# JokerYan/MS-GS

Hardware: AMD Instinct MI355X
Metric: Mpixels/s fwd+bwd @1080p, 1M Gaussians; fraction of HBM roofline (higher is better)
Workload: dtype f32

## Files before the change

### include/msgs.h

```cpp
#ifndef MSGS_H_
#define MSGS_H_

#include <stddef.h>
#include <stdint.h>

#ifdef __cplusplus
extern "C" {
#endif

#define MSGS_ABI_VERSION 11

#define MSGS_OK 0
#define MSGS_ERR_INVALID_ARG (-1)
#define MSGS_ERR_CAPACITY (-2)
#define MSGS_ERR_TOO_MANY (-3)
#define MSGS_ERR_SH_DEGREE (-4)
#define MSGS_ERR_INTERNAL (-5)
#define MSGS_ERR_NO_WEIGHT (-6)

#define MSGS_TILE 16

typedef struct msgs_view {
    int32_t image_height;
    int32_t image_width;
// ... 266 lines not shown
                            float* dL_dfeatures_dc, float* dL_dfeatures_rest, void* stream);

int msgs_mark_visible(int32_t P, const float* means3D, const float* viewmatrix,
                      const float* projmatrix, uint8_t* present, void* stream);

int msgs_binning_stats(const msgs_view_t* view, int32_t P, const int32_t* radii,
                       const void* binning, size_t binning_bytes,
                       const void* image_state, size_t image_bytes,
                       void* scratch, size_t scratch_bytes,
                       int64_t* out_host, void* stream);

int msgs_blend_lane_stats(const msgs_view_t* view, const void* geom, size_t geom_bytes, int32_t P, int64_t D,
                          const void* binning, size_t binning_bytes, const void* image_state, size_t image_bytes,
                          void* scratch, size_t scratch_bytes, int64_t* out_host, void* stream);

int msgs_set_deterministic(int32_t on);
int msgs_get_deterministic(void);
size_t msgs_backward_scratch_bytes_deterministic(int32_t P, int64_t D);
size_t msgs_backward_scratch_bytes_deterministic_depth(int32_t P, int64_t D);

int msgs_set_backward_generation(int32_t gen);

int msgs_set_blend_granularity(int32_t mode);

int msgs_set_occlusion(int32_t on);
int msgs_set_depth_sort(int32_t mode);
int msgs_depth_sort_stats(const void* geom, size_t geom_bytes, int32_t P, int64_t* out_host, void* stream);
int msgs_forward_info(int64_t* out_host);
int msgs_occlusion_stats(const void* geom, size_t geom_bytes, int32_t P, int64_t* out_host, void* stream);
int msgs_slab_stats(const void* geom, size_t geom_bytes, int32_t P, int64_t* out_host, void* stream);

int msgs_forward(const msgs_view_t* view, const msgs_gaussians_t* gaussians, int32_t* radii, float* pixel_sizes,
                 void* geom, size_t geom_bytes, void* scratch1, size_t scratch1_bytes, void* binning,
                 size_t binning_bytes, void* scratch2, size_t scratch2_bytes, void* image, size_t image_bytes,
                 float* out_color, float* out_acc_pixel_size, float* out_depth, void* grad_records,
                 size_t grad_records_bytes, int32_t backward_follows, int64_t* num_instances_host, int32_t* stage2_done,
                 const msgs_timing_t* timing, void* stream);

typedef struct msgs_status msgs_status_t;
int msgs_status_create(msgs_status_t** out);
int msgs_status_destroy(msgs_status_t* status);
int msgs_forward_launch(const msgs_view_t* view, const msgs_gaussians_t* gaussians, int32_t* radii, float* pixel_sizes,
                        void* geom, size_t geom_bytes, void* scratch1, size_t scratch1_bytes, void* binning,
                        size_t binning_bytes, void* scratch2, size_t scratch2_bytes, void* image, size_t image_bytes,
                        float* out_color, float* out_acc_pixel_size, float* out_depth, void* grad_records,
                        size_t grad_records_bytes, int32_t backward_follows, msgs_status_t* status,
// ... 226 lines not shown
```

### ms-gs_amd/csrc/api.hip

```cpp
#include "msgs_internal.h"

#include <atomic>
#include <new>

#include <cstring>

using namespace msgs;

namespace {

struct Timer {
    const msgs_timing_t* t;
    hipStream_t s;
    void begin(int k) const { if (t && t->ev[2 * k]) (void)hipEventRecord((hipEvent_t)t->ev[2 * k], s); }
    void end(int k) const { if (t && t->ev[2 * k + 1]) (void)hipEventRecord((hipEvent_t)t->ev[2 * k + 1], s); }
};

inline int check_inputs(const msgs_view_t* v, const msgs_gaussians_t* g) {
    if (!v || !g) return MSGS_ERR_INVALID_ARG;
    if (g->P < 0 || v->image_width <= 0 || v->image_height <= 0) return MSGS_ERR_INVALID_ARG;
    if (!v->bg || !v->viewmatrix || !v->projmatrix || !v->campos) return MSGS_ERR_INVALID_ARG;
    if (g->P > 0 && (!g->means3D || !g->opacities)) return MSGS_ERR_INVALID_ARG;
    if (g->raw_params) {
        if (g->raw_params != 1 && g->raw_params != 2) return MSGS_ERR_INVALID_ARG;
// ... 67 lines not shown
    const Stage2Scratch L(D);
    return L.total + align256(4 * (size_t)(D > 0 ? D : 1));
}
static int64_t tiles_of(int32_t W, int32_t H) { return (int64_t)((W + TILE - 1) / TILE) * ((H + TILE - 1) / TILE); }
size_t msgs_binning_bytes_slab(int64_t D, int32_t W, int32_t H, float fraction) {
    if (!(fraction > 0.f)) return msgs_binning_bytes(D, W, H);
    return msgs_binning_bytes(SlabGeom::ids_needed(D > 0 ? D : 1, (double)fraction, tiles_of(W, H)), W, H);
}
size_t msgs_stage2_scratch_bytes_slab(int64_t D, int32_t W, int32_t H) {
    return msgs_stage2_scratch_bytes((D > 0 ? D : 1) + SLAB_SLACK + 256, W, H);
}
size_t msgs_image_bytes(int32_t W, int32_t H) { return ImageLayout(W, H).total; }
size_t msgs_backward_scratch_bytes(int32_t P) {
    return align256(GRAD_REC_BYTES * (size_t)(P > 0 ? P : 1));
}
size_t msgs_backward_scratch_bytes_deterministic(int32_t P, int64_t D) { return DetScratch(P, D).total; }
size_t msgs_backward_scratch_bytes_deterministic_depth(int32_t P, int64_t D) { return DetScratch(P, D, DET_INST_FLOATS_DEPTH).total; }

static std::atomic<int> g_deterministic{[] { const char* e = getenv("MSGS_DETERMINISTIC"); return (e && e[0] == '1') ? 1 : 0; }()};
int msgs_set_deterministic(int32_t on) { return g_deterministic.exchange(on ? 1 : 0); }
int msgs_get_deterministic(void) { return g_deterministic.load(); }
int msgs_set_backward_generation(int32_t gen) { return set_backward_generation(gen); }
int msgs_set_blend_granularity(int32_t mode) { return set_blend_granularity(mode); }
int msgs_set_occlusion(int32_t on) { return set_occlusion(on); }
int msgs_set_depth_sort(int32_t mode) { return set_depth_sort(mode); }

}

namespace {
struct Stage2Buffers {
    void* binning; size_t binning_bytes;
    void* scratch2; size_t scratch2_bytes;
    void* image; size_t image_bytes;
    float* out_color; float* out_acc_ps; float* out_depth;
    void* grad_records; size_t grad_records_bytes;
    int backward_follows;
};

struct SpecStage2 {
    int64_t capacity;
    Stage2Buffers buf;
    int launched_rc;
};
int forward_stage2_impl(const msgs_view_t* view, const msgs_gaussians_t* g, const void* geom_v, size_t geom_bytes, int64_t D,
                        const Stage2Buffers& b, const msgs_timing_t* timing, void* stream, const uint32_t* D_dev,
                        uint64_t* fb_dev, uint64_t fb_ticket);
// ... 1487 lines not shown
```

### ms-gs_amd/csrc/blend.hip

```cpp
#include "msgs_internal.h"

#include <atomic>
#include <type_traits>

#include <algorithm>

namespace msgs {

namespace {

constexpr int BATCH = 256;
constexpr float ALPHA_MIN = 1.0f / 255.0f;
constexpr float T_MIN = 0.0001f;

struct PairEval { float dxx, dxy, dyy, p; };
__device__ __forceinline__ PairEval eval_pair(float A, float B2, float C, float lo, float dx, float dy) {
#pragma clang fp contract(off)
    PairEval e;
    e.dxx = __fmul_rn(dx, dx);
    e.dxy = __fmul_rn(dx, dy);
    e.dyy = __fmul_rn(dy, dy);
    e.p = __fmaf_rn(A, e.dxx, __fmaf_rn(B2, e.dxy, __fmaf_rn(C, e.dyy, lo)));
    return e;
}
__device__ __forceinline__ float4 doubled_w(const float4& r) { return make_float4(r.x, r.y, r.z, r.w + r.w); }
__device__ __forceinline__ float sign_test_bound(float lo) { return __fmaf_rn(fabsf(lo), 2.4e-7f, lo); }
__device__ __forceinline__ float4 with_bound(const float4& r2, float lo) { return make_float4(r2.x, r2.y, r2.z, sign_test_bound(lo)); }

__device__ __forceinline__ uint32_t quadrant_mask(const float4& r0, float C, float tau2, float tx0, float ty0) {
    if (!(tau2 > -1.0e38f)) return 0xFu;
    uint32_t m = 0;
#pragma unroll
    for (int q = 0; q < 4; ++q) {
        const float x0 = tx0 + (float)((q & 1) * 8), y0 = ty0 + (float)((q >> 1) * 8);
        if (levelset_hits_rect(r0.x, r0.y, r0.z, r0.w, C, tau2, x0, x0 + 7.0f, y0, y0 + 7.0f)) m |= 1u << q;
    }
    return m;
}

__device__ __forceinline__ int swizzled_tile(int bid, int num_tiles) {
    const int per = num_tiles >> 3;
    const int main = per << 3;
    if (bid >= main) return bid;
    return (bid & 7) * per + (bid >> 3);
}

constexpr int CLEAR_INLINE_MIN_TILES = 2048;
__device__ __forceinline__ void clear_slice(uint4* __restrict__ p, size_t n16) {
    if (p == nullptr) return;
// ... 381 lines not shown
                                               grad_acc_t* __restrict__ grad_rec, bool alane, uint32_t aoff) {
    const float outv = cross_row(row_reduce_scatter<DEPTH>(v, v9));
    const uint32_t gid = __builtin_amdgcn_readfirstlane(id());
    grad_acc_t* gdst = grad_rec + (size_t)gid * GRAD_REC_FLOATS;
    if (alane) unsafeAtomicAdd(gdst + aoff, (grad_acc_t)outv);
}
struct BwdPix {
    float T, S, dL0, dL1, dL2, dLd;
    uint32_t last;
};
template <bool ALPHA>
__device__ __forceinline__ void bwd_pix_start_S(BwdPix& st, const ViewParams& vp, bool inside, size_t pix,
                                                const float* dL_dalpha) {
    st.S = vp.bg[0] * st.dL0 + vp.bg[1] * st.dL1 + vp.bg[2] * st.dL2;
    if constexpr (ALPHA) { if (inside) st.S -= dL_dalpha[pix]; }
}
struct PairAlpha { PairEval ev; float a_raw; };
__device__ __forceinline__ PairAlpha pair_alpha(const float4& r0, const float4& r1, float dx, float dy) {
    PairAlpha a;
    a.ev = eval_pair(r0.z, r0.w, r1.x, r1.y, dx, dy);
    a.a_raw = __builtin_amdgcn_exp2f(a.ev.p);
    return a;
}
__device__ __forceinline__ uint64_t pair_valid(const PairAlpha& a, uint32_t pos, uint32_t last, float bound) {
    return __builtin_amdgcn_ballot_w64(pos < last) & __builtin_amdgcn_ballot_w64(a.ev.p <= bound) &
           __builtin_amdgcn_ballot_w64(a.a_raw >= ALPHA_MIN);
}
struct PairGrad { float q, dch; };
template <bool DEPTH, class Z>
__device__ __forceinline__ PairGrad pair_grad(BwdPix& s, const PairAlpha& a, uint64_t validm, const float4& r1, float cb, Z z) {
    const bool valid = __builtin_amdgcn_inverse_ballot_w64(validm);
    const float a_m = valid ? a.a_raw : 0.0f;
    const float alpha_m = fminf(0.99f, a_m);
    const float inv = __builtin_amdgcn_rcpf(1.0f - alpha_m);
    const float Tn = s.T * inv;
    s.T = Tn;
    PairGrad g;
    g.dch = alpha_m * Tn;
    float gi = fmaf(cb, s.dL2, fmaf(r1.w, s.dL1, r1.z * s.dL0));
    if constexpr (DEPTH) gi = fmaf(z(), s.dLd, gi);
    const float sm = gi - s.S;
    const float dL_dalpha = sm * Tn;
    s.S = fmaf(alpha_m, sm, s.S);
    g.q = a_m * dL_dalpha;
    return g;
}
template <bool CROSS_ROW, bool DEPTH = false>
__device__ __forceinline__ void backward_walk(const uint16_t* lp, int cnt, int base, const float4* s_r0, const float4* s_r1,
                                              const float2* s_b, const uint32_t* s_id, float pxf, float pyf, BwdPix& st,
                                              bool alane, uint32_t aoff, grad_acc_t* __restrict__ grad_rec,
                                              const float* s_z = nullptr) {
    for (int j = cnt - 1; j >= 0; --j) {
        const int e = lp[j];
        const float4 r0 = s_r0[e], r1 = s_r1[e];
        const float2 bl = s_b[e];
        const float dx = r0.x - pxf, dy = r0.y - pyf;
// ... 168 lines not shown
        if (b > 0) fetch(base - BATCH);
        __syncthreads();
        int cnt = 0;
#pragma unroll
        for (int c = 0; c < BATCH / 64; ++c) {
            const int e = c * 64 + lane;
            const bool hit = e < n && (uint32_t)(base + e) < wave_last && fine_hit<SB>(s_r0, s_r1, s_tau, e, bx0, by0);
            const uint64_t bal = __ballot(hit);
            if (hit) s_list[w][cnt + __popcll(bal & lt_mask)] = (uint16_t)e;
            cnt += __popcll(bal);
        }
        backward_walk<false, DEPTH>(s_list[w], cnt, base, s_r0, s_r1, s_b, s_id, pxf, pyf, st, alane, aoff, grad_rec, s_z);
    }
}

constexpr int WB = 64;

__device__ __forceinline__ void wave_fence() {
    __builtin_amdgcn_fence(__ATOMIC_RELEASE, "wavefront");
    __builtin_amdgcn_wave_barrier();
    __builtin_amdgcn_fence(__ATOMIC_ACQUIRE, "wavefront");
}

template <bool DEPTH>
__device__ __forceinline__ uint64_t bwd_quad_step(BwdPix& s, BwdSums& v, float* v9, const float4& r0, const float4& r1, float cb,
                                                  float bound, float dx, float dy, uint32_t pos0, float z) {
    const PairAlpha a = pair_alpha(r0, r1, dx, dy);
    const uint64_t validm = pair_valid(a, pos0, s.last, bound);
    const PairGrad g = pair_grad<DEPTH>(s, a, validm, r1, cb, [=] { return z; });
    v.v0 = fmaf(g.q, dx, v.v0); v.v1 = fmaf(g.q, dy, v.v1);
    v.v2 = fmaf(g.q, a.ev.dxx, v.v2); v.v3 = fmaf(g.q, a.ev.dxy, v.v3); v.v4 = fmaf(g.q, a.ev.dyy, v.v4);
    v.v5 += g.q;
    v.v6 = fmaf(g.dch, s.dL0, v.v6); v.v7 = fmaf(g.dch, s.dL1, v.v7); v.v8 = fmaf(g.dch, s.dL2, v.v8);
    if constexpr (DEPTH) *v9 = fmaf(g.dch, s.dLd, *v9);
    return validm;
}

#if defined(MSGS_TRACE_TILES)
__device__ unsigned long long* g_tile_trace = nullptr;
__global__ void trace_set_kernel(unsigned long long* p) { g_tile_trace = p; }
#endif

template <bool COUNT = false, int CH = 3, bool ALPHA = false>
__global__ __launch_bounds__(64) void blend_backward_tile_kernel(ViewParams vp, const GaussRec* __restrict__ rec,
                                                                 const uint32_t* __restrict__ ids,
                                                                 const uint2* __restrict__ ranges,
                                                                 const float* __restrict__ final_T,
                                                                 const uint32_t* __restrict__ n_contrib,
                                                                 const float* __restrict__ dL_dcolor,
                                                                 void* __restrict__ grad_out,
                                                                 const uint32_t* __restrict__ tile_order,
                                                                 const float* __restrict__ dL_ddepth,
                                                                 const float* __restrict__ dL_dalpha) {
    constexpr bool DEPTH = CH == 4;
    __shared__ float4 s_r0[WB], s_r1[WB];
    __shared__ float4 s_bi[WB];
    const int num_tiles = vp.gx * vp.gy;
    const int lane = threadIdx.x;
    int tile = swizzled_tile(blockIdx.x, num_tiles);
    if (tile_order != nullptr) {
        const uint32_t flag = tile_order[num_tiles];
        if (flag == TILE_ORDER_MAGIC) tile = (int)tile_order[tile];
    }
    const int tx = tile % vp.gx, ty = tile / vp.gx;
    const int bx = tx * TILE + (lane & 7), by = ty * TILE + (lane >> 3);
    const float bxf = (float)bx, byf = (float)by;
    const float tx0 = (float)(tx * TILE), ty0 = (float)(ty * TILE);
    const uint2 range = ranges[tile];
    const size_t N = (size_t)vp.W * vp.H;

#if defined(MSGS_TRACE_TILES)
    const unsigned long long trace_t0 = __builtin_amdgcn_s_memrealtime();
#endif
    uint32_t cnt_visits = 0, cnt_steps = 0, cnt_lanes = 0, cnt_hits = 0;
    BwdPix q0, q1, q2, q3;
    uint32_t ql0, ql1, ql2, ql3;
// ... 11 lines not shown
            s.S = vp.bg[0] * s.dL0 + vp.bg[1] * s.dL1 + vp.bg[2] * s.dL2;
            if constexpr (ALPHA) { if (inside) s.S -= dL_dalpha[pix]; }
            s.T = Tf;
            return __builtin_amdgcn_readfirstlane(wave_max_u32(s.last));
        };
        ql0 = init(q0, 0); ql1 = init(q1, 1); ql2 = init(q2, 2); ql3 = init(q3, 3);
    }
    const uint32_t tile_last = max(max(ql0, ql1), max(ql2, ql3));
    const bool alane = IS_ATOMIC_LANE(DEPTH, lane);
    const uint32_t aoff = row_reduce_component<DEPTH>(lane);
    const int xrow16 = (lane ^ 16) << 2, xrow32 = (lane ^ 32) << 2;

    const int nb = ((int)tile_last + WB - 1) / WB;
    float4 n0 = make_float4(0, 0, 0, 0), n1 = n0, n2 = n0;
    uint32_t nid = 0;
    if (nb > 0) {
        const int i0 = (nb - 1) * WB + lane;
        if (i0 < (int)tile_last) { nid = ids[range.x + i0]; n0 = rec[nid].r0; n1 = rec[nid].r1; n2 = rec[nid].r2; }
    }
    for (int b = nb - 1; b >= 0; --b) {
        const int base = b * WB;
        const int n = min(WB, (int)tile_last - base);
        wave_fence();
        s_r0[lane] = doubled_w(n0); s_r1[lane] = n1; s_bi[lane] = make_float4(n2.x, sign_test_bound(n1.y), __uint_as_float(nid), DEPTH ? n2.y : 0.f);
        const uint32_t mymask = lane < n ? quadrant_mask(n0, n1.x, n2.w, tx0, ty0) : 0u;
        const uint32_t mypos = (uint32_t)(base + lane);
        const uint64_t h0 = __ballot((mymask & 1u) && mypos < ql0), h1 = __ballot((mymask & 2u) && mypos < ql1),
                       h2 = __ballot((mymask & 4u) && mypos < ql2), h3 = __ballot((mymask & 8u) && mypos < ql3);
        wave_fence();
        if (b > 0) {
            nid = ids[range.x + base - WB + lane];
            n0 = rec[nid].r0; n1 = rec[nid].r1; n2 = rec[nid].r2;
        }
        uint64_t todo = h0 | h1 | h2 | h3;
        while (todo) {
            const int e = 63 - __builtin_clzll(todo);
            const uint64_t bit = 1ull << e;
            todo &= ~bit;
            const uint32_t pos0 = (uint32_t)(base + e);
            const float4 r0 = s_r0[e], r1 = s_r1[e];
            const float2 bl = *reinterpret_cast<const float2*>(&s_bi[e]);
            const float dx = r0.x - bxf, dy = r0.y - byf;
            BwdSums v = {0, 0, 0, 0, 0, 0, 0, 0, 0};
            float v9 = 0.f;
            float* const pv9 = DEPTH ? &v9 : nullptr;
            const float z = DEPTH ? s_bi[e].w : 0.f;
            uint64_t any = 0;
            if constexpr (COUNT) cnt_visits += 1u;
            if (h0 & bit) {
                const uint64_t m = bwd_quad_step<DEPTH>(q0, v, pv9, r0, r1, bl.x, bl.y, dx, dy, pos0, z);
                any |= m;
                if constexpr (COUNT) { cnt_steps += 1u; cnt_lanes += (uint32_t)__popcll(m); }
            }
            if (h1 & bit) {
                const uint64_t m = bwd_quad_step<DEPTH>(q1, v, pv9, r0, r1, bl.x, bl.y, dx - 8.0f, dy, pos0, z);
                any |= m;
                if constexpr (COUNT) { cnt_steps += 1u; cnt_lanes += (uint32_t)__popcll(m); }
            }
            if (h2 & bit) {
                const uint64_t m = bwd_quad_step<DEPTH>(q2, v, pv9, r0, r1, bl.x, bl.y, dx, dy - 8.0f, pos0, z);
                any |= m;
                if constexpr (COUNT) { cnt_steps += 1u; cnt_lanes += (uint32_t)__popcll(m); }
            }
            if (h3 & bit) {
                const uint64_t m = bwd_quad_step<DEPTH>(q3, v, pv9, r0, r1, bl.x, bl.y, dx - 8.0f, dy - 8.0f, pos0, z);
                any |= m;
                if constexpr (COUNT) { cnt_steps += 1u; cnt_lanes += (uint32_t)__popcll(m); }
            }
            if constexpr (COUNT) {
                if (any) cnt_hits += 1u;
                continue;
            }
            if (any == 0) continue;
            reduce_and_add<DEPTH>(v, v9, [=](float x) { return cross_row_allreduce_bperm(x, xrow16, xrow32); },
                                  [=] { return __float_as_uint(s_bi[e].z); }, (grad_acc_t*)grad_out, alane, aoff);
        }
    }
    if constexpr (COUNT) {
        if (lane == 0) {
            unsigned long long* o = (unsigned long long*)grad_out;
            atomicAdd(&o[0], (unsigned long long)cnt_visits); atomicAdd(&o[1], (unsigned long long)cnt_steps);
            atomicAdd(&o[2], (unsigned long long)cnt_lanes); atomicAdd(&o[3], (unsigned long long)cnt_hits);
        }
    }
#if defined(MSGS_TRACE_TILES)
    if (!COUNT && !DEPTH && g_tile_trace && lane == 0) {
        unsigned hw, xcc;
        asm volatile("s_getreg_b32 %0, hwreg(HW_REG_HW_ID)" : "=s"(hw));
        asm volatile("s_getreg_b32 %0, hwreg(HW_REG_XCC_ID)" : "=s"(xcc));
        unsigned long long* o = g_tile_trace + 4ull * blockIdx.x;
        o[0] = trace_t0; o[1] = __builtin_amdgcn_s_memrealtime();
        o[2] = ((unsigned long long)xcc << 32) | hw; o[3] = ((unsigned long long)tile << 32) | tile_last;
    }
#endif
}

struct ReplayPixel {
    int tile, tx, ty, tid, w, lane, px, py;
// ... 661 lines not shown
    const uint32_t v = (px < vp.W && py < vp.H) ? n_contrib[(size_t)py * vp.W + px] : 0u;
    const uint32_t m = wave_max_u32(v);
    if (lane == 0) s_wmax[w] = m;
    __syncthreads();
    if (tid == 0) atomicAdd(&out[0], (unsigned long long)max(max(s_wmax[0], s_wmax[1]), max(s_wmax[2], s_wmax[3])));
}

__global__ __launch_bounds__(256) void visible_count_kernel(int P, const int32_t* __restrict__ radii,
                                                            unsigned long long* __restrict__ out) {
    const int i = blockIdx.x * blockDim.x + threadIdx.x;
    const bool vis = i < P && radii[i] > 0;
    const uint64_t b = __ballot(vis);
    if ((threadIdx.x & 63) == 0 && b) atomicAdd(&out[1], (unsigned long long)__popcll(b));
}

}

constexpr int BWD_GEN2_MIN_TILES = 4096;
constexpr int FINE_MAX_TILES_FWD = 300, FINE_MAX_TILES_BWD = 300;
static std::atomic<int> g_bwd_gen{[] { const char* e = getenv("MSGS_BWD_GEN"); return (e && (e[0] == '1' || e[0] == '2')) ? e[0] - '0' : 0; }()};
int set_backward_generation(int gen) { return g_bwd_gen.exchange(gen == 1 || gen == 2 ? gen : 0); }
static std::atomic<int> g_granularity{[] { const char* e = getenv("MSGS_BLEND_GRANULARITY"); return (e && (e[0] == '1' || e[0] == '2')) ? e[0] - '0' : 0; }()};
int set_blend_granularity(int mode) { return g_granularity.exchange(mode == 1 || mode == 2 ? mode : 0); }
template <int WAVES, int SB>
struct FineShape { static constexpr int waves = WAVES, sb = SB, groups = (TILE / SB) * (TILE / SB) / WAVES; };
template <class F>
static void with_fine_shape(int tiles, F&& f) {
    if (tiles <= 16) f(FineShape<4, 1>{});
    else if (tiles <= 64) f(FineShape<4, 2>{});
    else if (tiles < 768) f(FineShape<4, 4>{});
    else f(FineShape<16, 4>{});
}

enum class FwdRoute { Quadrant, Fine };
enum class BwdRoute { Fine, Quadrant, Tile };
struct Routes { FwdRoute fwd; BwdRoute bwd; };
static Routes routes(int tiles) {
    const int gran = g_granularity.load(), gen = g_bwd_gen.load();
    Routes r;
    r.fwd = gran == 2 || (gran == 0 && tiles < FINE_MAX_TILES_FWD) ? FwdRoute::Fine : FwdRoute::Quadrant;
    if (gran == 2 || (gran == 0 && gen == 0 && tiles < FINE_MAX_TILES_BWD)) r.bwd = BwdRoute::Fine;
    else r.bwd = (gen ? gen == 1 : tiles < BWD_GEN2_MIN_TILES) ? BwdRoute::Quadrant : BwdRoute::Tile;
    return r;
}

namespace {
// ... 100 lines not shown
}

bool forward_uses_quadrant_kernel(int tiles) { return tiles > 0 && routes(tiles).fwd == FwdRoute::Quadrant; }

hipError_t launch_blend_backward(const ViewParams& vp, const char* geom, const uint32_t* ids, const uint2* ranges,
                                 const float* final_T, const uint32_t* n_contrib, const float* dL_dcolor,
                                 grad_acc_t* grad_rec, hipStream_t s, const uint32_t* tile_order, const float* dL_ddepth,
                                 const float* dL_dalpha) {
    const int tiles = vp.gx * vp.gy;
    if (tiles == 0) return hipSuccess;
    const GaussRec* rec = reinterpret_cast<const GaussRec*>(geom);
    const BwdRoute route = routes(tiles).bwd;
    with_bool(dL_ddepth != nullptr, [&](auto DEPTH) { with_bool(dL_dalpha != nullptr, [&](auto ALPHA) {
        constexpr int CH = decltype(DEPTH)::value ? 4 : 3;
        constexpr bool AL = decltype(ALPHA)::value;
        if (route == BwdRoute::Fine)
            with_fine_shape(tiles, [&](auto shape) {
                using S = decltype(shape);
                hipLaunchKernelGGL((blend_backward_fine_kernel<S::waves, S::sb, CH, AL>), dim3(tiles * S::groups), dim3(64 * S::waves), 0, s,
                                   vp, rec, ids, ranges, final_T, n_contrib, dL_dcolor, grad_rec, dL_ddepth, dL_dalpha);
            });
        else if (route == BwdRoute::Tile)
            hipLaunchKernelGGL((blend_backward_tile_kernel<false, CH, AL>), dim3(tiles), dim3(64), 0, s, vp, rec, ids, ranges, final_T,
                               n_contrib, dL_dcolor, (void*)grad_rec, tile_order, dL_ddepth, dL_dalpha);
        else
            hipLaunchKernelGGL((blend_backward_kernel<CH, AL>), dim3(tiles), dim3(256), 0, s, vp, rec, ids, ranges, final_T, n_contrib,
                               dL_dcolor, grad_rec, dL_ddepth, dL_dalpha);
    }); });
    return hipGetLastError();
}

hipError_t launch_blend_absgrad(const ReplayInputs& in, int P, const float* dL_dcolor, const float* dL_ddepth,
                                const float* dL_dalpha, double* acc, float* out, hipStream_t s) {
    const int tiles = in.vp.gx * in.vp.gy;
    hipError_t e = launch_zero(acc, 2 * sizeof(double) * (size_t)P, s);
    if (e != hipSuccess) return e;
    if (tiles > 0)
        with_bool(dL_ddepth != nullptr, [&](auto DEPTH) { with_bool(dL_dalpha != nullptr, [&](auto ALPHA) {
            hipLaunchKernelGGL((blend_absgrad_kernel<decltype(DEPTH)::value, decltype(ALPHA)::value>), dim3(tiles), dim3(256), 0, s,
                               in.vp, in.rec, in.ids, in.ranges, in.final_T, in.n_contrib, dL_dcolor, acc, dL_ddepth, dL_dalpha);
        }); });
    constexpr float LN2 = 0.69314718055994530942f;
    hipLaunchKernelGGL(absgrad_finish_kernel, dim3((P + 255) / 256), dim3(256), 0, s, P, LN2 * in.vp.W, LN2 * in.vp.H,
                       (const double*)acc, out);
    return hipGetLastError();
}

// ... 132 lines not shown
    if (e != hipSuccess) return e;
    int bits = 1;
    while (bits < 32 && ((int64_t)1 << bits) < P) ++bits;
    e = radix_sort_pairs(keys, nullptr, keys_s, entry, D, 0, bits, scratch + L.sort, s);
    if (e != hipSuccess) return e;
    static_assert(sizeof(grad_acc_t) == 8, "the verification mode's sums are doubles");
    static_assert(DET_INST_FLOATS_DEPTH <= GRAD_REC_FLOATS, "the [P, 10] sums fit the grad_rec region");
    with_bool(dL_ddepth != nullptr, [&](auto DEPTH) {
        constexpr int NF = decltype(DEPTH)::value ? DET_INST_FLOATS_DEPTH : DET_INST_FLOATS;
        hipLaunchKernelGGL(det_reduce_kernel<NF>, dim3((unsigned)((D + 255) / 256)), dim3(256), 0, s, keys_s, entry, D, inst, grad_rec, NF);
    });
    return hipGetLastError();
}

hipError_t launch_blend_backward_lane_stats(const ViewParams& vp, const char* geom, const uint32_t* ids, const uint2* ranges,
                                            const float* final_T, const uint32_t* n_contrib, unsigned long long* out4,
                                            hipStream_t s) {
    hipError_t e = hipMemsetAsync(out4, 0, 32, s);
    if (e != hipSuccess) return e;
    const int tiles = vp.gx * vp.gy;
    if (tiles)
        hipLaunchKernelGGL(blend_backward_tile_kernel<true>, dim3(tiles), dim3(64), 0, s, vp,
                           reinterpret_cast<const GaussRec*>(geom), ids, ranges, final_T, n_contrib, (const float*)nullptr, (void*)out4,
                           (const uint32_t*)nullptr, (const float*)nullptr, (const float*)nullptr);
    return hipGetLastError();
}

hipError_t launch_blend_lane_stats(const ViewParams& vp, const char* geom, const uint32_t* ids, const uint2* ranges,
                                   unsigned long long* out3, hipStream_t s) {
    hipError_t e = hipMemsetAsync(out3, 0, 24, s);
    if (e != hipSuccess) return e;
    const int tiles = vp.gx * vp.gy;
    if (tiles)
        hipLaunchKernelGGL(blend_forward_kernel<true>, dim3(tiles), dim3(256), 0, s, vp, reinterpret_cast<const GaussRec*>(geom),
                           ids, ranges, (float*)nullptr, (float*)nullptr, (float*)nullptr, (float*)nullptr,
                           (uint32_t*)nullptr, out3, (uint4*)nullptr, (size_t)0, (uint32_t*)nullptr, (uint32_t*)nullptr,
                           FwdSlab{nullptr, nullptr, nullptr, nullptr, nullptr, nullptr});
    return hipGetLastError();
}

hipError_t launch_binning_stats(const ViewParams& vp, int P, const int32_t* radii, const uint32_t* n_contrib,
                                unsigned long long* out2, hipStream_t s) {
    hipError_t e = hipMemsetAsync(out2, 0, 16, s);
    if (e != hipSuccess) return e;
    const int tiles = vp.gx * vp.gy;
    if (tiles) hipLaunchKernelGGL(tile_stats_kernel, dim3(tiles), dim3(256), 0, s, vp, n_contrib, out2);
    if (P) hipLaunchKernelGGL(visible_count_kernel, dim3((P + 255) / 256), dim3(256), 0, s, P, radii, out2);
    return hipGetLastError();
}

}

#if defined(MSGS_TRACE_TILES)
extern "C" int msgs_debug_set_tile_trace(void* p) {
    hipLaunchKernelGGL(msgs::trace_set_kernel, dim3(1), dim3(1), 0, 0, (unsigned long long*)p);
    return (int)hipDeviceSynchronize();
}
#endif
```

### ms-gs_amd/csrc/msgs_internal.h

```cpp
#pragma once
#include <hip/hip_runtime.h>
#include <stdint.h>
#include <cmath>
#include <type_traits>
#include "../../include/msgs.h"

namespace msgs {

constexpr int TILE = MSGS_TILE;
constexpr int WAVE = 64;

struct __attribute__((aligned(16))) GaussRec { float4 r0, r1, r2; };

struct __attribute__((aligned(32))) BinRec { float4 q0, q1; };

#if defined(MSGS_GRAD_REC_F32)
typedef float grad_acc_t;
constexpr int GRAD_REC_FLOATS = 12;
#else
typedef double grad_acc_t;
constexpr int GRAD_REC_FLOATS = 10;
#endif
constexpr uint32_t TILE_ORDER_MAGIC = 0x4C505431u;
constexpr size_t GRAD_REC_BYTES = sizeof(grad_acc_t) * GRAD_REC_FLOATS;
// ... 529 lines not shown
                              uint64_t* status = nullptr, uint64_t* host_mapped = nullptr, uint64_t ticket = 0,
                              const uint32_t* n_ptr = nullptr, uint32_t* clamped_total = nullptr, uint64_t clamp = 0,
                              const uint32_t* extra = nullptr,
                              uint32_t* zero_word = nullptr,
                              uint32_t* overflow_flag = nullptr, uint32_t in_mask = 0xFFFFFFFFu, uint32_t* side_out = nullptr,
                              uint32_t* side_flag = nullptr);
template <class F>
inline void with_bool(bool b, F&& f) {
    if (b) f(std::true_type{}); else f(std::false_type{});
}
hipError_t launch_zero(void* ptr, size_t bytes, hipStream_t s);
hipError_t launch_emit(const ViewParams& vp, int P, const char* geom, uint32_t* keys, uint32_t* ids,
                       int64_t D, hipStream_t s, ZeroJob zj = ZeroJob{nullptr, 0, nullptr, 0}, const uint32_t* D_dev = nullptr,
                       bool keys16 = false, uint32_t* heavy_q = nullptr, int slab = 0, const uint32_t* open_bits = nullptr,
                       int64_t density_D = 0);
hipError_t launch_slab_split(int P, char* geom, int64_t D, const uint32_t* D_dev, float fraction, uint32_t* open_bits,
                             int num_tiles, hipStream_t s);
hipError_t launch_slab_recount(const ViewParams& vp, int P, char* geom, const uint32_t* open_bits, const uint32_t* open_list, int64_t D,
                               const uint32_t* D_dev, hipStream_t s);
hipError_t launch_ranges(const uint32_t* keys, int64_t D, uint2* ranges, int num_tiles, hipStream_t s,
                         bool pre_zeroed = false, const uint32_t* D_dev = nullptr, bool keys16 = false, uint32_t base = 0);
int set_backward_generation(int gen);
int set_blend_granularity(int mode);
struct DetScratch {
    size_t grad_rec, inst_grad, keys, keys_s, entry, sort, total;
    DetScratch(int64_t P, int64_t D, int nf = DET_INST_FLOATS);
};
hipError_t launch_blend_backward_det(const ViewParams& vp, int P, const char* geom, const uint32_t* ids, int64_t D,
                                     const uint2* ranges, const float* final_T, const uint32_t* n_contrib,
                                     const float* dL_dcolor, char* scratch, hipStream_t s, const float* dL_ddepth = nullptr,
                                     const float* dL_dalpha = nullptr);

hipError_t launch_alpha_map(const float* final_T, float* out_alpha, size_t N, hipStream_t s);
size_t bg_grad_rows_bytes(size_t N);
hipError_t launch_bg_grad(const float* final_T , const float* dL_dcolor, size_t N, float* dL_dbg,
                          double* rows, hipStream_t s);

hipError_t launch_adam(const msgs_adam_tensor_t* tensors, int n, int64_t step, double beta1, double beta2, double eps,
                       hipStream_t s);
hipError_t launch_densify_stats(const msgs_densify_stats_t& d, hipStream_t s);

size_t densify_scratch_bytes(int64_t P, int64_t n_append);
int densify_check_select(const msgs_densify_select_t& s);
int densify_check_apply(const msgs_densify_apply_t& a);
int densify_select(const msgs_densify_select_t& s, char* scratch, int64_t* counts_host, hipStream_t st);
int densify_apply(const msgs_densify_apply_t& a, const char* scratch, hipStream_t st);
// ... 116 lines not shown
```

### ms-gs_amd/diff_gaussian_rasterization/__init__.py

```python
import ctypes as C
import os
import threading
import weakref
from typing import NamedTuple

import torch
import torch.nn as nn

from . import _backend as _C

__all__ = ["GaussianRasterizationSettings", "GaussianRasterizer", "rasterize_gaussians", "rasterize_gaussians_raw",
           "deferred_forward", "GradAccumulator", "set_grad_accumulator", "ContributionScores", "ContributionAccumulator",
           "screen_compensation", "compute_3d_filter", "smoothing_filter", "FILTER3D_CAMERA_CHUNK",
           "gaussian_normals", "depth_to_normal", "DEPTH_NORMAL_TILE_W", "DEPTH_NORMAL_TILE_H",
           "bilateral_slice", "total_variation_loss", "BILAGRID_TILE_W", "BILAGRID_TILE_H", "BILAGRID_WINDOW_CELLS",
           "tsdf_allocate", "tsdf_integrate", "tsdf_extract", "tsdf_mark_steps", "TSDF_CAMERA_CHUNK", "TSDF_MAX_BLOCKS_PER_AXIS",
           "TSDF_MAX_SLOTS"]


class GaussianRasterizationSettings(NamedTuple):
    image_height: int
    image_width: int
    tanfovx: float
    tanfovy: float
# ... 508 lines not shown
        raise ValueError("camera gradients (a viewmatrix / projmatrix / campos that requires grad) cannot be combined with "
                         "set_optimizer_in_backward")
    if _sinks.sh_factor[0] is not None:
        raise ValueError("camera gradients (a viewmatrix / projmatrix / campos that requires grad) cannot be combined with "
                         "the factored SH gradient of the view-parallel exchange")


class _CameraGrads:

    def __init__(self, ctx, P, dev):
        vm, pm, cp = ctx.camera
        self.dV = torch.empty(16, dtype=torch.float32, device=dev) if vm is not None else None
        self.dPM = torch.empty(16, dtype=torch.float32, device=dev) if pm is not None else None
        self.dcp = torch.empty(3, dtype=torch.float32, device=dev) if cp is not None else None
        self.scratch = _bytes(_C.lib.msgs_camera_grad_scratch_bytes(P), dev)

    def grads(self, ctx):
        return tuple(None if m is None else g.view(m[0]).to(device=m[2], dtype=m[1])
                     for g, m in zip((self.dV, self.dPM, self.dcp), ctx.camera))


def set_deterministic(on=True):
    return bool(_C.lib.msgs_set_deterministic(1 if on else 0))


class _LRU(dict):

    def __init__(self, cap=256):
        super().__init__()
        self.cap = cap

    def __setitem__(self, k, v):
        if k in self:
            super().__delitem__(k)
        super().__setitem__(k, v)
        while len(self) > self.cap:
            super().__delitem__(next(iter(self)))

    def setdefault(self, k, default=None):
        if k not in self:
            self[k] = default
        return self[k]


_last_instances = _LRU()
_instances_by_view = _LRU()
# ... 1637 lines not shown
```

### ms-gs_amd/diff_gaussian_rasterization/_backend.py

```python
import ctypes as C
import os
import threading

import torch

_PKG = os.path.dirname(os.path.abspath(__file__))
_LIB_PATH = os.environ.get("MSGS_HIP_LIB") or next(
    (p for p in (os.path.join(_PKG, "libmsgs_hip.so"),) if os.path.exists(p)),
    os.path.join(os.path.dirname(_PKG), "lib", "libmsgs_hip.so"))

ABI_VERSION = 11

K_NAMES = ("preprocess", "depth_sort", "scan", "emit", "tile_sort", "ranges", "blend_fwd", "blend_bwd",
           "preprocess_bwd", "slab_b")
K_COUNT = len(K_NAMES)


class View(C.Structure):
    _fields_ = [("image_height", C.c_int32), ("image_width", C.c_int32),
                ("tanfovx", C.c_float), ("tanfovy", C.c_float),
                ("scale_modifier", C.c_float), ("fade_size", C.c_float),
                ("sh_degree", C.c_int32), ("sh_coeffs", C.c_int32),
                ("filter_small", C.c_int32), ("filter_large", C.c_int32),
                ("prefiltered", C.c_int32), ("debug", C.c_int32),
# ... 142 lines not shown
                       ("msgs_backward_scratch_bytes", [C.c_int32])):
        f = getattr(lib, name)
        f.restype = sz
        f.argtypes = args
    lib.msgs_forward_stage1.restype = C.c_int
    lib.msgs_forward_stage1.argtypes = [C.POINTER(View), C.POINTER(Gaussians), vp, vp, vp, sz, vp, sz,
                                        C.POINTER(C.c_int64), C.POINTER(Timing), vp]
    lib.msgs_set_deterministic.restype = C.c_int
    lib.msgs_set_deterministic.argtypes = [C.c_int32]
    lib.msgs_get_deterministic.restype = C.c_int
    lib.msgs_get_deterministic.argtypes = []
    lib.msgs_backward_scratch_bytes_deterministic.restype = sz
    lib.msgs_backward_scratch_bytes_deterministic.argtypes = [C.c_int32, C.c_int64]
    lib.msgs_backward_scratch_bytes_deterministic_depth.restype = sz
    lib.msgs_backward_scratch_bytes_deterministic_depth.argtypes = [C.c_int32, C.c_int64]
    lib.msgs_set_backward_generation.restype = C.c_int
    lib.msgs_set_backward_generation.argtypes = [C.c_int32]
    lib.msgs_set_blend_granularity.restype = C.c_int
    lib.msgs_set_blend_granularity.argtypes = [C.c_int32]
    lib.msgs_forward_info.restype = C.c_int
    lib.msgs_forward_info.argtypes = [C.POINTER(C.c_int64)]
    lib.msgs_set_occlusion.restype = C.c_int
    lib.msgs_set_occlusion.argtypes = [C.c_int32]
    lib.msgs_occlusion_stats.restype = C.c_int
    lib.msgs_occlusion_stats.argtypes = [vp, sz, C.c_int32, C.POINTER(C.c_int64), vp]
    lib.msgs_set_depth_sort.restype = C.c_int
    lib.msgs_set_depth_sort.argtypes = [C.c_int32]
    lib.msgs_depth_sort_stats.restype = C.c_int
    lib.msgs_depth_sort_stats.argtypes = [vp, sz, C.c_int32, C.POINTER(C.c_int64), vp]
    lib.msgs_slab_stats.restype = C.c_int
    lib.msgs_slab_stats.argtypes = [vp, sz, C.c_int32, C.POINTER(C.c_int64), vp]
    lib.msgs_forward.restype = C.c_int
    lib.msgs_forward.argtypes = [C.POINTER(View), C.POINTER(Gaussians), vp, vp, vp, sz, vp, sz, vp, sz, vp, sz, vp, sz,
                                 vp, vp, vp, vp, sz, C.c_int32, C.POINTER(C.c_int64), C.POINTER(C.c_int32), C.POINTER(Timing), vp]
    lib.msgs_status_create.restype = C.c_int
    lib.msgs_status_create.argtypes = [C.POINTER(vp)]
    lib.msgs_status_destroy.restype = C.c_int
    lib.msgs_status_destroy.argtypes = [vp]
    lib.msgs_forward_launch.restype = C.c_int
    lib.msgs_forward_launch.argtypes = [C.POINTER(View), C.POINTER(Gaussians), vp, vp, vp, sz, vp, sz, vp, sz, vp, sz, vp, sz,
                                        vp, vp, vp, vp, sz, C.c_int32, vp, C.POINTER(Timing), vp]
    lib.msgs_forward_finish.restype = C.c_int
    lib.msgs_forward_finish.argtypes = [vp, C.POINTER(C.c_int64), C.POINTER(C.c_int32)]
    lib.msgs_preprocess_only.restype = C.c_int
    lib.msgs_preprocess_only.argtypes = [C.POINTER(View), C.POINTER(Gaussians), vp, vp, vp, sz, vp]
    lib.msgs_forward_stage2.restype = C.c_int
# ... 162 lines not shown
           "msgs_get_deterministic", "msgs_backward_scratch_bytes_deterministic",
           "msgs_set_backward_generation", "msgs_set_blend_granularity", "msgs_sh_grad_from_views",
           "msgs_blend_lane_stats", "msgs_backward_per_gaussian",
           "msgs_status_create", "msgs_status_destroy", "msgs_forward_launch", "msgs_forward_finish",
           "msgs_set_occlusion", "msgs_occlusion_stats", "msgs_forward_info", "msgs_binning_bytes_slab",
           "msgs_stage2_scratch_bytes_slab", "msgs_slab_stats", "msgs_backward_with_depth",
           "msgs_backward_scratch_bytes_deterministic_depth", "msgs_backward_with_camera", "msgs_camera_grad_scratch_bytes",
           "msgs_densify_scratch_bytes", "msgs_densify_select", "msgs_densify_apply",
           "msgs_alpha_map", "msgs_backward_with_alpha", "msgs_bg_grad_scratch_bytes", "msgs_bg_grad",
           "msgs_absgrad_scratch_bytes", "msgs_absgrad",
           "msgs_contrib_scratch_bytes", "msgs_contrib_accumulate", "msgs_contrib_finish",
           "msgs_features_scratch_bytes", "msgs_features_forward", "msgs_features_backward",
           "msgs_distortion_forward", "msgs_distortion_backward",
           "msgs_median_depth_forward", "msgs_median_depth_backward",
           "msgs_screen_compensation_forward", "msgs_screen_compensation_backward", "msgs_screen_compensation_scratch_bytes",
           "msgs_filter3d_scratch_bytes", "msgs_filter3d_sweep", "msgs_smoothing_filter_forward",
           "msgs_smoothing_filter_backward",
           "msgs_gaussian_normals_forward", "msgs_gaussian_normals_backward", "msgs_depth_normal_forward",
           "msgs_depth_normal_backward",
           "msgs_bilagrid_scratch_bytes", "msgs_bilagrid_slice_forward", "msgs_bilagrid_slice_backward",
           "msgs_bilagrid_tv_scratch_bytes", "msgs_bilagrid_tv_forward", "msgs_bilagrid_tv_backward",
           "msgs_mcmc_scratch_bytes", "msgs_mcmc_prepare", "msgs_mcmc_sample", "msgs_mcmc_relocate", "msgs_mcmc_noise",
           "msgs_tsdf_mark_blocks", "msgs_tsdf_integrate", "msgs_tsdf_count", "msgs_tsdf_emit",
           "msgs_set_depth_sort", "msgs_depth_sort_stats")


def check(rc, where):
    if rc == 0:
        return
    msg = lib.msgs_error_string(int(rc)).decode()
    if rc in (-1, -4):
        raise ValueError(f"{where}: {msg}")
    raise RuntimeError(f"{where}: error {rc}: {msg}")


class KernelTimer:

    def __init__(self, only=None):
        self.t = Timing()
        check(lib.msgs_timing_create(C.byref(self.t)), "msgs_timing_create")
        self.active = self.t
        if only is not None:
            self.active = Timing()
            for k, name in enumerate(K_NAMES):
                if name in only:
                    self.active.ev[2 * k], self.active.ev[2 * k + 1] = self.t.ev[2 * k], self.t.ev[2 * k + 1]

# ... 26 lines not shown
```

Baseline: 2016.

## Specialise backward tile blend for tame Gaussians, skipping bound test and alpha clamp

Adds a per-record 'tame' classification (bounded conic, non-degenerate quadratic form, log2 opacity below a limit) computed when a batch is staged. Runs of tame records are visited through a template specialisation that drops the sign-test ballot and the 0.99 alpha clamp. The first quad step writes its accumulators directly instead of adding to zeroed values. The aim is fewer VALU ops and ballots per Gaussian-pixel pair in the backward tile kernel, in exchange for extra classification work per batch, more code and register pressure from two instantiations, and reliance on the proof that the skipped checks are redundant. Host-side helpers for validating the exp2 bound are also added.

Measured after the change: 2036, median of 6. Within noise of the previous version (+1.0%).

```diff
diff --git a/include/msgs.h b/include/msgs.h
--- a/include/msgs.h
+++ b/include/msgs.h
@@ -312,6 +312,11 @@
 int msgs_set_backward_generation(int32_t gen);
 
 int msgs_set_blend_granularity(int32_t mode);
+
+int msgs_set_blend_specialise(int32_t on);
+int msgs_blend_record_tame(float A, float B2, float C, float log2_opacity);
+float msgs_blend_tame_log2_limit(void);
+int msgs_blend_exp2_max(float x_hi, float x_lo, uint32_t* out_host2, void* stream);
 
 int msgs_set_occlusion(int32_t on);
 int msgs_set_depth_sort(int32_t mode);
diff --git a/ms-gs_amd/csrc/api.hip b/ms-gs_amd/csrc/api.hip
--- a/ms-gs_amd/csrc/api.hip
+++ b/ms-gs_amd/csrc/api.hip
@@ -113,6 +113,21 @@
 int msgs_get_deterministic(void) { return g_deterministic.load(); }
 int msgs_set_backward_generation(int32_t gen) { return set_backward_generation(gen); }
 int msgs_set_blend_granularity(int32_t mode) { return set_blend_granularity(mode); }
+int msgs_set_blend_specialise(int32_t on) { return set_blend_specialise(on); }
+int msgs_blend_record_tame(float A, float B2, float C, float log2_opacity) { return blend_record_tame(A, B2, C, log2_opacity); }
+float msgs_blend_tame_log2_limit(void) { return blend_tame_log2_limit(); }
+int msgs_blend_exp2_max(float x_hi, float x_lo, uint32_t* out_host2, void* stream) {
+    if (!out_host2) return (int)hipErrorInvalidValue;
+    hipStream_t s = (hipStream_t)stream;
+    uint32_t* d = nullptr;
+    hipError_t e = hipMalloc((void**)&d, 8);
+    if (e != hipSuccess) return (int)e;
+    e = launch_exp2_max(x_hi, x_lo, d, s);
+    if (e == hipSuccess) e = hipMemcpyAsync(out_host2, d, 8, hipMemcpyDeviceToHost, s);
+    if (e == hipSuccess) e = hipStreamSynchronize(s);
+    (void)hipFree(d);
+    return (int)e;
+}
 int msgs_set_occlusion(int32_t on) { return set_occlusion(on); }
 int msgs_set_depth_sort(int32_t mode) { return set_depth_sort(mode); }
 
diff --git a/ms-gs_amd/csrc/blend.hip b/ms-gs_amd/csrc/blend.hip
--- a/ms-gs_amd/csrc/blend.hip
+++ b/ms-gs_amd/csrc/blend.hip
@@ -1,6 +1,8 @@
 #include "msgs_internal.h"
+#include "blend_tame.h"
 
 #include <atomic>
+#include <cstring>
 #include <type_traits>
 
 #include <algorithm>
@@ -24,7 +26,6 @@
     return e;
 }
 __device__ __forceinline__ float4 doubled_w(const float4& r) { return make_float4(r.x, r.y, r.z, r.w + r.w); }
-__device__ __forceinline__ float sign_test_bound(float lo) { return __fmaf_rn(fabsf(lo), 2.4e-7f, lo); }
 __device__ __forceinline__ float4 with_bound(const float4& r2, float lo) { return make_float4(r2.x, r2.y, r2.z, sign_test_bound(lo)); }
 
 __device__ __forceinline__ uint32_t quadrant_mask(const float4& r0, float C, float tau2, float tx0, float ty0) {
@@ -452,16 +453,19 @@
     a.a_raw = __builtin_amdgcn_exp2f(a.ev.p);
     return a;
 }
+template <bool TAME = false>
 __device__ __forceinline__ uint64_t pair_valid(const PairAlpha& a, uint32_t pos, uint32_t last, float bound) {
+    if constexpr (TAME)
+        return __builtin_amdgcn_ballot_w64(pos < last) & __builtin_amdgcn_ballot_w64(a.a_raw >= ALPHA_MIN);
     return __builtin_amdgcn_ballot_w64(pos < last) & __builtin_amdgcn_ballot_w64(a.ev.p <= bound) &
            __builtin_amdgcn_ballot_w64(a.a_raw >= ALPHA_MIN);
 }
 struct PairGrad { float q, dch; };
-template <bool DEPTH, class Z>
+template <bool DEPTH, bool TAME = false, class Z>
 __device__ __forceinline__ PairGrad pair_grad(BwdPix& s, const PairAlpha& a, uint64_t validm, const float4& r1, float cb, Z z) {
     const bool valid = __builtin_amdgcn_inverse_ballot_w64(validm);
     const float a_m = valid ? a.a_raw : 0.0f;
-    const float alpha_m = fminf(0.99f, a_m);
+    const float alpha_m = TAME ? a_m : fminf(0.99f, a_m);
     const float inv = __builtin_amdgcn_rcpf(1.0f - alpha_m);
     const float Tn = s.T * inv;
     s.T = Tn;
@@ -676,17 +680,25 @@
     __builtin_amdgcn_fence(__ATOMIC_ACQUIRE, "wavefront");
 }
 
-template <bool DEPTH>
+template <bool DEPTH, bool FIRST, bool TAME>
 __device__ __forceinline__ uint64_t bwd_quad_step(BwdPix& s, BwdSums& v, float* v9, const float4& r0, const float4& r1, float cb,
                                                   float bound, float dx, float dy, uint32_t pos0, float z) {
     const PairAlpha a = pair_alpha(r0, r1, dx, dy);
-    const uint64_t validm = pair_valid(a, pos0, s.last, bound);
-    const PairGrad g = pair_grad<DEPTH>(s, a, validm, r1, cb, [=] { return z; });
-    v.v0 = fmaf(g.q, dx, v.v0); v.v1 = fmaf(g.q, dy, v.v1);
-    v.v2 = fmaf(g.q, a.ev.dxx, v.v2); v.v3 = fmaf(g.q, a.ev.dxy, v.v3); v.v4 = fmaf(g.q, a.ev.dyy, v.v4);
-    v.v5 += g.q;
-    v.v6 = fmaf(g.dch, s.dL0, v.v6); v.v7 = fmaf(g.dch, s.dL1, v.v7); v.v8 = fmaf(g.dch, s.dL2, v.v8);
-    if constexpr (DEPTH) *v9 = fmaf(g.dch, s.dLd, *v9);
+    const uint64_t validm = pair_valid<TAME>(a, pos0, s.last, bound);
+    const PairGrad g = pair_grad<DEPTH, TAME>(s, a, validm, r1, cb, [=] { return z; });
+    if constexpr (FIRST) {
+        v.v0 = fmaf(g.q, dx, 0.0f); v.v1 = fmaf(g.q, dy, 0.0f);
+        v.v2 = fmaf(g.q, a.ev.dxx, 0.0f); v.v3 = fmaf(g.q, a.ev.dxy, 0.0f); v.v4 = fmaf(g.q, a.ev.dyy, 0.0f);
+        v.v5 = 0.0f + g.q;
+        v.v6 = fmaf(g.dch, s.dL0, 0.0f); v.v7 = fmaf(g.dch, s.dL1, 0.0f); v.v8 = fmaf(g.dch, s.dL2, 0.0f);
+        if constexpr (DEPTH) *v9 = fmaf(g.dch, s.dLd, 0.0f);
+    } else {
+        v.v0 = fmaf(g.q, dx, v.v0); v.v1 = fmaf(g.q, dy, v.v1);
+        v.v2 = fmaf(g.q, a.ev.dxx, v.v2); v.v3 = fmaf(g.q, a.ev.dxy, v.v3); v.v4 = fmaf(g.q, a.ev.dyy, v.v4);
+        v.v5 += g.q;
+        v.v6 = fmaf(g.dch, s.dL0, v.v6); v.v7 = fmaf(g.dch, s.dL1, v.v7); v.v8 = fmaf(g.dch, s.dL2, v.v8);
+        if constexpr (DEPTH) *v9 = fmaf(g.dch, s.dLd, *v9);
+    }
     return validm;
 }
 
@@ -705,7 +717,7 @@
                                                                  void* __restrict__ grad_out,
                                                                  const uint32_t* __restrict__ tile_order,
                                                                  const float* __restrict__ dL_ddepth,
-                                                                 const float* __restrict__ dL_dalpha) {
+                                                                 const float* __restrict__ dL_dalpha, int specialise) {
     constexpr bool DEPTH = CH == 4;
     __shared__ float4 s_r0[WB], s_r1[WB];
     __shared__ float4 s_bi[WB];
@@ -763,7 +775,10 @@
         const int base = b * WB;
         const int n = min(WB, (int)tile_last - base);
         wave_fence();
-        s_r0[lane] = doubled_w(n0); s_r1[lane] = n1; s_bi[lane] = make_float4(n2.x, sign_test_bound(n1.y), __uint_as_float(nid), DEPTH ? n2.y : 0.f);
+        const float4 st0 = doubled_w(n0);
+        const float nbound = sign_test_bound(n1.y);
+        s_r0[lane] = st0; s_r1[lane] = n1; s_bi[lane] = make_float4(n2.x, nbound, __uint_as_float(nid), DEPTH ? n2.y : 0.f);
+        const uint64_t tame = (!COUNT && specialise) ? __ballot(lane < n && record_tame(st0.z, st0.w, n1.x, nbound)) : 0ull;
         const uint32_t mymask = lane < n ? quadrant_mask(n0, n1.x, n2.w, tx0, ty0) : 0u;
         const uint32_t mypos = (uint32_t)(base + lane);
         const uint64_t h0 = __ballot((mymask & 1u) && mypos < ql0), h1 = __ballot((mymask & 2u) && mypos < ql1),
@@ -773,48 +788,53 @@
             nid = ids[range.x + base - WB + lane];
             n0 = rec[nid].r0; n1 = rec[nid].r1; n2 = rec[nid].r2;
         }
-        uint64_t todo = h0 | h1 | h2 | h3;
-        while (todo) {
-            const int e = 63 - __builtin_clzll(todo);
+        auto visit = [&](auto tame_c, int e) {
+            constexpr bool TM = decltype(tame_c)::value;
             const uint64_t bit = 1ull << e;
-            todo &= ~bit;
             const uint32_t pos0 = (uint32_t)(base + e);
             const float4 r0 = s_r0[e], r1 = s_r1[e];
             const float2 bl = *reinterpret_cast<const float2*>(&s_bi[e]);
             const float dx = r0.x - bxf, dy = r0.y - byf;
-            BwdSums v = {0, 0, 0, 0, 0, 0, 0, 0, 0};
-            float v9 = 0.f;
+            BwdSums v;
+            float v9;
             float* const pv9 = DEPTH ? &v9 : nullptr;
             const float z = DEPTH ? s_bi[e].w : 0.f;
+            if constexpr (COUNT) cnt_visits += 1u;
+            auto step = [&](auto first_c, BwdPix& q, float sdx, float sdy) -> uint64_t {
+                const uint64_t m = bwd_quad_step<DEPTH, decltype(first_c)::value, TM>(q, v, pv9, r0, r1, bl.x, bl.y, sdx, sdy, pos0, z);
+                if constexpr (COUNT) { cnt_steps += 1u; cnt_lanes += (uint32_t)__popcll(m); }
+                return m;
+            };
+            constexpr std::false_type later{};
             uint64_t any = 0;
-            if constexpr (COUNT) cnt_visits += 1u;
-            if (h0 & bit) {
-                const uint64_t m = bwd_quad_step<DEPTH>(q0, v, pv9, r0, r1, bl.x, bl.y, dx, dy, pos0, z);
-                any |= m;
-                if constexpr (COUNT) { cnt_steps += 1u; cnt_lanes += (uint32_t)__popcll(m); }
-            }
-            if (h1 & bit) {
-                const uint64_t m = bwd_quad_step<DEPTH>(q1, v, pv9, r0, r1, bl.x, bl.y, dx - 8.0f, dy, pos0, z);
-                any |= m;
-                if constexpr (COUNT) { cnt_steps += 1u; cnt_lanes += (uint32_t)__popcll(m); }
-            }
-            if (h2 & bit) {
-                const uint64_t m = bwd_quad_step<DEPTH>(q2, v, pv9, r0, r1, bl.x, bl.y, dx, dy - 8.0f, pos0, z);
-                any |= m;
-                if constexpr (COUNT) { cnt_steps += 1u; cnt_lanes += (uint32_t)__popcll(m); }
-            }
-            if (h3 & bit) {
-                const uint64_t m = bwd_quad_step<DEPTH>(q3, v, pv9, r0, r1, bl.x, bl.y, dx - 8.0f, dy - 8.0f, pos0, z);
-                any |= m;
-                if constexpr (COUNT) { cnt_steps += 1u; cnt_lanes += (uint32_t)__popcll(m); }
-            }
+            if (h0 & bit) any = step(std::true_type{}, q0, dx, dy);
+            else { v = BwdSums{0, 0, 0, 0, 0, 0, 0, 0, 0}; v9 = 0.f; }
+            if (h1 & bit) any |= step(later, q1, dx - 8.0f, dy);
+            if (h2 & bit) any |= step(later, q2, dx, dy - 8.0f);
+            if (h3 & bit) any |= step(later, q3, dx - 8.0f, dy - 8.0f);
             if constexpr (COUNT) {
                 if (any) cnt_hits += 1u;
-                continue;
+                return;
             }
-            if (any == 0) continue;
+            if (any == 0) return;
             reduce_and_add<DEPTH>(v, v9, [=](float x) { return cross_row_allreduce_bperm(x, xrow16, xrow32); },
                                   [=] { return __float_as_uint(s_bi[e].z); }, (grad_acc_t*)grad_out, alane, aoff);
+        };
+        uint64_t todo = h0 | h1 | h2 | h3;
+        while (todo) {
+            const uint64_t general = todo & ~tame;
+            uint64_t run = general ? todo & ~((2ull << (63 - __builtin_clzll(general))) - 1ull) : todo;
+            todo &= ~run;
+            while (run) {
+                const int e = 63 - __builtin_clzll(run);
+                run &= ~(1ull << e);
+                visit(std::true_type{}, e);
+            }
+            if (todo) {
+                const int e = 63 - __builtin_clzll(todo);
+                todo &= ~(1ull << e);
+                visit(std::false_type{}, e);
+            }
         }
     }
     if constexpr (COUNT) {
@@ -1522,6 +1542,8 @@
 int set_backward_generation(int gen) { return g_bwd_gen.exchange(gen == 1 || gen == 2 ? gen : 0); }
 static std::atomic<int> g_granularity{[] { const char* e = getenv("MSGS_BLEND_GRANULARITY"); return (e && (e[0] == '1' || e[0] == '2')) ? e[0] - '0' : 0; }()};
 int set_blend_granularity(int mode) { return g_granularity.exchange(mode == 1 || mode == 2 ? mode : 0); }
+static std::atomic<int> g_specialise{[] { const char* e = getenv("MSGS_BLEND_SPECIALISE"); return (e && e[0] == '0') ? 0 : 1; }()};
+int set_blend_specialise(int on) { return g_specialise.exchange(on ? 1 : 0); }
 template <int WAVES, int SB>
 struct FineShape { static constexpr int waves = WAVES, sb = SB, groups = (TILE / SB) * (TILE / SB) / WAVES; };
 template <class F>
@@ -1668,7 +1690,7 @@
             });
         else if (route == BwdRoute::Tile)
             hipLaunchKernelGGL((blend_backward_tile_kernel<false, CH, AL>), dim3(tiles), dim3(64), 0, s, vp, rec, ids, ranges, final_T,
-                               n_contrib, dL_dcolor, (void*)grad_rec, tile_order, dL_ddepth, dL_dalpha);
+                               n_contrib, dL_dcolor, (void*)grad_rec, tile_order, dL_ddepth, dL_dalpha, g_specialise.load());
         else
             hipLaunchKernelGGL((blend_backward_kernel<CH, AL>), dim3(tiles), dim3(256), 0, s, vp, rec, ids, ranges, final_T, n_contrib,
                                dL_dcolor, grad_rec, dL_ddepth, dL_dalpha);
@@ -1847,7 +1869,7 @@
     if (tiles)
         hipLaunchKernelGGL(blend_backward_tile_kernel<true>, dim3(tiles), dim3(64), 0, s, vp,
                            reinterpret_cast<const GaussRec*>(geom), ids, ranges, final_T, n_contrib, (const float*)nullptr, (void*)out4,
-                           (const uint32_t*)nullptr, (const float*)nullptr, (const float*)nullptr);
+                           (const uint32_t*)nullptr, (const float*)nullptr, (const float*)nullptr, 0);
     return hipGetLastError();
 }
 
@@ -1874,6 +1896,33 @@
     return hipGetLastError();
 }
 
+namespace {
+__global__ __launch_bounds__(256) void exp2_max_kernel(uint32_t bits_first, uint32_t bits_last, uint32_t* __restrict__ out2) {
+    const uint64_t total = (uint64_t)bits_last - bits_first + 1u;
+    uint32_t best = 0u, count = 0u;
+    for (uint64_t i = (uint64_t)blockIdx.x * blockDim.x + threadIdx.x; i < total; i += (uint64_t)gridDim.x * blockDim.x) {
+        const float y = __builtin_amdgcn_exp2f(__uint_as_float(bits_first + (uint32_t)i));
+        best = max(best, __float_as_uint(y));
+        count += 1u;
+    }
+    best = wave_max_u32(best);
+    for (int o = 32; o > 0; o >>= 1) count += __shfl_xor(count, o);
+    if ((threadIdx.x & 63) == 0) { atomicMax(&out2[0], best); atomicAdd(&out2[1], count); }
+}
+}
+
+float blend_tame_log2_limit() { return TAME_LOG2_LIMIT; }
+int blend_record_tame(float A, float B2, float C, float lo) { return record_tame(A, B2, C, sign_test_bound(lo)) ? 1 : 0; }
+hipError_t launch_exp2_max(float x_hi, float x_lo, uint32_t* out2, hipStream_t s) {
+    if (!(x_lo <= x_hi) || !(x_hi < 0.f)) return hipErrorInvalidValue;
+    hipError_t e = hipMemsetAsync(out2, 0, 8, s);
+    if (e != hipSuccess) return e;
+    uint32_t first, last;
+    memcpy(&first, &x_hi, 4); memcpy(&last, &x_lo, 4);
+    hipLaunchKernelGGL(exp2_max_kernel, dim3(2048), dim3(256), 0, s, first, last, out2);
+    return hipGetLastError();
+}
+
 }
 
 #if defined(MSGS_TRACE_TILES)
diff --git a/ms-gs_amd/csrc/blend_tame.h b/ms-gs_amd/csrc/blend_tame.h
--- /dev/null
+++ b/ms-gs_amd/csrc/blend_tame.h
@@ -0,0 +1,27 @@
+#pragma once
+
+#include <cmath>
+
+#if defined(__HIPCC__)
+#define MSGS_TAME_HD __host__ __device__ __forceinline__
+#else
+#define MSGS_TAME_HD inline
+#endif
+
+namespace msgs {
+
+MSGS_TAME_HD float sign_test_bound(float lo) { return fmaf(fabsf(lo), 2.4e-7f, lo); }
+
+constexpr float TAME_K = 3.9990234375f;
+constexpr float TAME_CONIC_MIN = 9.094947017729282e-13f, TAME_CONIC_MAX = 1099511627776.0f;
+constexpr float TAME_LOG2_LIMIT = -0.0146f;
+
+MSGS_TAME_HD bool record_tame(float A, float B2, float C, float bound) {
+    const float a = -A, c = -C;
+    const float bb = B2 * B2, ac = A * C;
+    const float k = TAME_K * ac;
+    return a >= TAME_CONIC_MIN && a <= TAME_CONIC_MAX && c >= TAME_CONIC_MIN && c <= TAME_CONIC_MAX && bb <= k &&
+           bound <= TAME_LOG2_LIMIT;
+}
+
+}
diff --git a/ms-gs_amd/csrc/msgs_internal.h b/ms-gs_amd/csrc/msgs_internal.h
--- a/ms-gs_amd/csrc/msgs_internal.h
+++ b/ms-gs_amd/csrc/msgs_internal.h
@@ -575,6 +575,10 @@
                          bool pre_zeroed = false, const uint32_t* D_dev = nullptr, bool keys16 = false, uint32_t base = 0);
 int set_backward_generation(int gen);
 int set_blend_granularity(int mode);
+int set_blend_specialise(int on);
+int blend_record_tame(float A, float B2, float C, float lo);
+float blend_tame_log2_limit();
+hipError_t launch_exp2_max(float x_hi, float x_lo, uint32_t* out2, hipStream_t s);
 struct DetScratch {
     size_t grad_rec, inst_grad, keys, keys_s, entry, sort, total;
     DetScratch(int64_t P, int64_t D, int nf = DET_INST_FLOATS);
diff --git a/ms-gs_amd/diff_gaussian_rasterization/__init__.py b/ms-gs_amd/diff_gaussian_rasterization/__init__.py
--- a/ms-gs_amd/diff_gaussian_rasterization/__init__.py
+++ b/ms-gs_amd/diff_gaussian_rasterization/__init__.py
@@ -554,6 +554,10 @@
 
 def set_deterministic(on=True):
     return bool(_C.lib.msgs_set_deterministic(1 if on else 0))
+
+
+def set_blend_specialise(on=True):
+    return bool(_C.lib.msgs_set_blend_specialise(1 if on else 0))
 
 
 class _LRU(dict):
diff --git a/ms-gs_amd/diff_gaussian_rasterization/_backend.py b/ms-gs_amd/diff_gaussian_rasterization/_backend.py
--- a/ms-gs_amd/diff_gaussian_rasterization/_backend.py
+++ b/ms-gs_amd/diff_gaussian_rasterization/_backend.py
@@ -188,6 +188,14 @@
     lib.msgs_forward_info.argtypes = [C.POINTER(C.c_int64)]
     lib.msgs_set_occlusion.restype = C.c_int
     lib.msgs_set_occlusion.argtypes = [C.c_int32]
+    lib.msgs_set_blend_specialise.restype = C.c_int
+    lib.msgs_set_blend_specialise.argtypes = [C.c_int32]
+    lib.msgs_blend_record_tame.restype = C.c_int
+    lib.msgs_blend_record_tame.argtypes = [C.c_float, C.c_float, C.c_float, C.c_float]
+    lib.msgs_blend_tame_log2_limit.restype = C.c_float
+    lib.msgs_blend_tame_log2_limit.argtypes = []
+    lib.msgs_blend_exp2_max.restype = C.c_int
+    lib.msgs_blend_exp2_max.argtypes = [C.c_float, C.c_float, C.POINTER(C.c_uint32), vp]
     lib.msgs_occlusion_stats.restype = C.c_int
     lib.msgs_occlusion_stats.argtypes = [vp, sz, C.c_int32, C.POINTER(C.c_int64), vp]
     lib.msgs_set_depth_sort.restype = C.c_int
@@ -396,7 +404,8 @@
            "msgs_bilagrid_tv_scratch_bytes", "msgs_bilagrid_tv_forward", "msgs_bilagrid_tv_backward",
            "msgs_mcmc_scratch_bytes", "msgs_mcmc_prepare", "msgs_mcmc_sample", "msgs_mcmc_relocate", "msgs_mcmc_noise",
            "msgs_tsdf_mark_blocks", "msgs_tsdf_integrate", "msgs_tsdf_count", "msgs_tsdf_emit",
-           "msgs_set_depth_sort", "msgs_depth_sort_stats")
+           "msgs_set_depth_sort", "msgs_depth_sort_stats",
+           "msgs_set_blend_specialise", "msgs_blend_record_tame", "msgs_blend_tame_log2_limit", "msgs_blend_exp2_max")
 
 
 def check(rc, where):
```
